# leducthanhig/image-restoration-models

Hardware: AMD Instinct MI355X
Metric: images/sec + PSNR, Restormer motion-deblur 1280x720 (higher is better)
Workload: dtype f32 (1x1 convs: fp32 emulated by 3 fp16 MFMAs on hi/lo operand splits with fp32 accumulation, error vs float64 at the level of an fp32 chain; everything else exact f32; value_exact_f32: f32 MFMA everywhere); 1 GPU; Restormer motion-deblur (WithBias LN, 26.13M params, synthetic weights seed 42) on 1280x720x3 uint8 GoPro-shaped synthetic frames; 6 tiles 512x512 (overlap 96) per frame; a step = 4 frame(s) per GPU, their 24 tiles in one batched forward; global_batch=4, tile=512, overlap=96, parallelism=per-image shard x1, no data-path collective

## Files before the change

### image-restoration-models_amd/csrc/fused_tail.hip

```cpp
#include "irm_common.h"

struct TailArgs {
    const float* Hh; long h_bs;
    float* X; long x_bs;
    const float* rec;
    const float* w2;
    const float* bias2;
    int C, H, W, S, HP, CB;
    float inv_s2;
    int tiles_x, tiles, items, gpx;
};

template <int CT>
__global__ __launch_bounds__(512, 2) void gdfn_tail_kernel(TailArgs a) {
    constexpr int RECF = 512;
    constexpr int W2F = CT * 512, W2P = CT * 2;
    constexpr int SLOT_B = RECF * 4, W2_OFF = 2 * SLOT_B, PL_OFF = W2_OFF + W2F * 4, PL_B = IRM_PLF * 4;
    constexpr int PARK_OFF = PL_OFF + 2 * PL_B;
    constexpr int NK = (IRM_NP * 8 + 511) / 512;
    static_assert(PARK_OFF + 8192 <= 160 * 1024, "LDS");
    extern __shared__ __attribute__((aligned(16))) float smem[];
    irm_lc* lds = (irm_lc*)smem;
    float* slots = smem;
    float* w2a = smem + W2_OFF / 4;

    const int wave = __builtin_amdgcn_readfirstlane((int)threadIdx.x >> 6);
    const long plane = (long)a.H * a.W;
    const int S = a.S;
    const int per = (a.items + 7) >> 3;
    const int xcd = blockIdx.x & 7, pos = blockIdx.x >> 3;
    auto item_of = [&](int round) { const int i = round * a.gpx + pos; return i < per ? xcd * per + i : a.items; };

    int round = 0;
    int item = item_of(0);
    if (item >= a.items) return;

    for (;;) {
        int tid = threadIdx.x;
        asm volatile("" : "+v"(tid));
        const int lane = tid & 63, g = lane >> 4, r = lane & 15;
        const int b = item / a.tiles, tile = item - b * a.tiles;
        const int ty0 = (tile / a.tiles_x) * IRM_TH, tx0 = (tile % a.tiles_x) * IRM_TW;
        const float* Hh = a.Hh + (long)b * a.h_bs;
        const unsigned vw = irm_opaque((unsigned)(lane * 16));
        const unsigned vc = irm_opaque((unsigned)(16 * g));
        const int sp0 = (2 * (wave >> 1)) * IRM_HC + 16 * (wave & 1) + r;
        const unsigned vp0 = irm_opaque((unsigned)(PL_OFF + (sp0 * IRM_PS + 4 * g) * 4));
        const unsigned vp1 = irm_opaque(vp0 + PL_B);

        int goff[NK];
        unsigned loff[NK];
#pragma unroll
        for (int k = 0; k < NK; ++k) {
            const int idx = k * 512 + tid, px = idx >> 3, pc = idx & 7;
            const int hr = px / IRM_HC, hc = px - hr * IRM_HC;
            const int gy = ty0 - 1 + hr, gx = tx0 - 1 + hc;
            const bool valid = px < IRM_NP, inside = valid && gy >= 0 && gy < a.H && gx >= 0 && gx < a.W;
            goff[k] = inside ? ((gy >> 3) * a.tiles_x + (gx >> 5)) * 256 * a.CB + ((gy & 7) * IRM_TW + (gx & 31)) * 64 + (pc & 3) * 4 +
                               (pc >> 2) * (a.HP / 64) * (256 * 64)
                             : -1;
            loff[k] = (unsigned)(PL_OFF + ((valid ? px : IRM_NP + (tid & 15)) * IRM_PS) * 4 + (pc & 3) * 16 + (pc >> 2) * 64);
        }
        f32x4 hreg[NK];
        const float* const zero_page = irm_zero_page;
        auto load_h = [&](int s) {
#pragma unroll
            for (int k = 0; k < NK; ++k) {
                const float* src = goff[k] >= 0 ? Hh + goff[k] + (s >> 2) * (256 * 64) + (s & 3) * 16 : zero_page;
                hreg[k] = *reinterpret_cast<const f32x4*>(src);
            }
        };
        auto park_h = [&](int img) {
#pragma unroll
            for (int k = 0; k < NK; ++k) irm_st<f32x4>(lds, loff[k], img * PL_B, hreg[k]);
        };

        const int nitem = item_of(round + 1);

        irm_dma<2>(a.rec, slots, wave, lane);
        irm_dma<W2P>(a.w2, w2a, wave, lane);
        load_h(0);
        f32x4 acc2[2][CT];
        const unsigned vpark = irm_opaque((unsigned)(PARK_OFF + threadIdx.x * 16));
#pragma unroll
        for (int c = 0; c < CT; ++c) { acc2[0][c] = (f32x4){0.f, 0.f, 0.f, 0.f}; acc2[1][c] = (f32x4){0.f, 0.f, 0.f, 0.f}; }
        irm_st<f32x4>(lds, vpark, 0, acc2[1][CT - 1]);
        park_h(0);
        asm volatile("s_waitcnt vmcnt(0) lgkmcnt(0)" ::: "memory");
        __builtin_amdgcn_s_barrier();

        float o[2][2][4];
        f32x4 kprev[3];

        irm_u4 Gh[2], Gl[2];
#pragma unroll
        for (int q = 0; q < 2; ++q) { Gh[q] = (irm_u4){0u, 0u, 0u, 0u}; Gl[q] = (irm_u4){0u, 0u, 0u, 0u}; }

        auto iter = [&](auto PAR, auto MORE, int it) {
            constexpr int par = decltype(PAR)::value;
            constexpr bool more = decltype(MORE)::value;
            if constexpr (more) {
                load_h(it + 1);
                irm_dma<2>(a.rec + (long)(it + 1) * RECF, slots + (par ^ 1) * RECF, wave, lane);
            }
            if (par == 0 && it > 0) irm_dma<W2P>(a.w2 + (long)(it >> 1) * W2F, w2a, wave, lane);
            {
                const unsigned vp = par ? vp1 : vp0;
                f32x4 P[2][3], K[2][3], KB[1];
                auto loads = [&](auto IC, auto NC) {
                    constexpr int I = decltype(IC)::value, n = decltype(NC)::value;
                    constexpr int hf = I >> 2, dy = I & 3;
                    constexpr int cf = par * SLOT_B + hf * 64;
                    if constexpr (dy == 0) irm_dsr<cf + 9 * 128>(KB[0], vc);
                    if constexpr (dy < 3) {
                        irm_dsr<cf + (dy * 3 + 0) * 128>(K[n][0], vc);
                        irm_dsr<cf + (dy * 3 + 1) * 128>(K[n][1], vc);
                        irm_dsr<cf + (dy * 3 + 2) * 128>(K[n][2], vc);
                    }
                    irm_dsr<(dy * IRM_HC + 0) * (IRM_PS * 4) + hf * 64>(P[n][0], vp);
                    irm_dsr<(dy * IRM_HC + 1) * (IRM_PS * 4) + hf * 64>(P[n][1], vp);
                    irm_dsr<(dy * IRM_HC + 2) * (IRM_PS * 4) + hf * 64>(P[n][2], vp);
                };
                loads(irm_ic<0>{}, irm_ic<0>{});
                irm_for<8>([&](auto IC) {
                    constexpr int I = decltype(IC)::value, c = I & 1, n = c ^ 1;
                    constexpr int hf = I >> 2, dy = I & 3;
                    if constexpr (I + 1 < 8) loads(irm_ic<I + 1>{}, irm_ic<n>{});
                    constexpr int J = I + 1, jdy = J & 3;
                    constexpr int nnext = J < 8 ? 3 + (jdy < 3 ? 3 : 0) + (jdy == 0 ? 1 : 0) : 0;
                    irm_wait_lgkmcnt<nnext>();
                    irm_tie(P[c][0], P[c][1], P[c][2]);
                    if constexpr (dy < 3) irm_tie(K[c][0], K[c][1], K[c][2]);
                    if constexpr (dy == 0) irm_tie(KB[0]);
                    irm_stencil_step(dy, o[hf], kprev, P[c], K[c], KB[0]);
                    __builtin_amdgcn_sched_barrier(0);
                });
            }
#pragma unroll
            for (int q = 0; q < 2; ++q)
#pragma unroll
                for (int e = 0; e < 4; e += 2) {
                    unsigned hh, ll;
                    irm_gate_split2(o[0][q][e], o[0][q][e + 1], o[1][q][e], o[1][q][e + 1], hh, ll);
                    Gh[q][2 * par + e / 2] = hh;
                    Gl[q][2 * par + e / 2] = ll;
                }
#pragma unroll
            for (int q = 0; q < 2; ++q) asm volatile("" : "+v"(Gh[q]), "+v"(Gl[q]));
            if (par == 1 || !more) {
                if constexpr (par == 0) {
                    asm volatile("s_waitcnt vmcnt(0)" ::: "memory");
                    __builtin_amdgcn_s_barrier();
                }
                f32x4 accp = irm_ld<f32x4>(lds, vpark, 0);
#pragma unroll
                for (int c = 0; c < CT; ++c) {
                    const irm_h8 bh = irm_ld<irm_h8>(lds, vw, W2_OFF + (c * 2) * 1024);
                    const irm_h8 bl = irm_ld<irm_h8>(lds, vw, W2_OFF + (c * 2 + 1) * 1024);
#pragma unroll
                    for (int q = 0; q < 2; ++q) {
                        f32x4& t = (q == 1 && c == CT - 1) ? accp : acc2[q][c];
                        t = irm_mfma3_f16(__builtin_bit_cast(irm_h8, Gh[q]), __builtin_bit_cast(irm_h8, Gl[q]), bh, bl, t);
                    }
                }
                irm_st<f32x4>(lds, vpark, 0, accp);
#pragma unroll
                for (int q = 0; q < 2; ++q) { Gh[q] = (irm_u4){0u, 0u, 0u, 0u}; Gl[q] = (irm_u4){0u, 0u, 0u, 0u}; }
            }
            if constexpr (more) park_h(par ^ 1);
            asm volatile("s_waitcnt vmcnt(0) lgkmcnt(0)" ::: "memory");
            __builtin_amdgcn_s_barrier();
        };
        {
            const std::integral_constant<int, 0> P0; const std::integral_constant<int, 1> P1;
            const std::true_type T; const std::false_type F;
            int it = 0;
            for (; it + 2 < S; it += 2) { iter(P0, T, it); iter(P1, T, it + 1); }
            if (it + 2 == S) { iter(P0, T, it); iter(P1, F, it + 1); }
            else iter(P0, F, it);
        }

        {
            int t3 = threadIdx.x;
            asm volatile("" : "+v"(t3));
            const int r3 = t3 & 15, ox = tx0 + 16 * (wave & 1) + 4 * ((t3 & 63) >> 4), oy0 = ty0 + 2 * (wave >> 1);
            float* X = a.X + (long)b * a.x_bs;
            acc2[1][CT - 1] = irm_ld<f32x4>(lds, vpark, 0);
#pragma unroll
            for (int c = 0; c < CT; ++c) {
                const int co = 16 * c + r3;
                if (co >= a.C || ox >= a.W) continue;
                const float bv = a.bias2 ? a.bias2[co] : 0.0f;
#pragma unroll
                for (int q = 0; q < 2; ++q) {
                    if (oy0 + q >= a.H) continue;
                    float4* px = reinterpret_cast<float4*>(X + (long)co * plane + (long)(oy0 + q) * a.W + ox);
                    const float4 xv = *px;
                    *px = make_float4(fmaf(acc2[q][c][0], a.inv_s2, xv.x + bv), fmaf(acc2[q][c][1], a.inv_s2, xv.y + bv),
                                      fmaf(acc2[q][c][2], a.inv_s2, xv.z + bv), fmaf(acc2[q][c][3], a.inv_s2, xv.w + bv));
                }
            }
        }
        if (nitem >= a.items) break;
        item = nitem;
        ++round;
    }
}

extern "C" int irm_gdfn_tail_f16x3_f32(const float* h_cl, long h_bs, const float* rec, const float* w2, const float* bias2,
                                       float* x, long x_bs, float inv_s2, int B, int C, int hid, int hid_pad, int H, int W,
                                       hipStream_t stream) {
    if (!h_cl || !rec || !w2 || !x || B <= 0 || C <= 0 || hid <= 0 || H <= 0 || W <= 0) return IRM_EINVAL;
    if (C != 192 || (H & 7) || (W & 31) || hid_pad < hid || (hid_pad & 63)) return IRM_EINVAL;
    if ((h_bs & 3) || (x_bs & 3) || !irm_aligned16(h_cl) || !irm_aligned16(x) || !irm_aligned16(rec) || !irm_aligned16(w2)) return IRM_EINVAL;
    if ((long)(H / 8) * (W / 32) * 256 * 2 * hid_pad >= (1L << 31)) return IRM_EINVAL;
    TailArgs a;
    a.Hh = h_cl; a.h_bs = h_bs; a.X = x; a.x_bs = x_bs; a.rec = rec; a.w2 = w2; a.bias2 = bias2;
    a.C = C; a.H = H; a.W = W; a.S = (hid + 15) / 16; a.HP = hid_pad; a.CB = 2 * hid_pad; a.inv_s2 = inv_s2;
    a.tiles_x = W / IRM_TW; a.tiles = a.tiles_x * (H / IRM_TH); a.items = B * a.tiles;
    constexpr int CT = 12;
    const size_t lds = (size_t)(2 * 512 + CT * 512 + 2 * IRM_PLF + 2048) * sizeof(float);
    IRM_ALLOW_BIG_LDS((&gdfn_tail_kernel<CT>));
    int dev = 0, n = 0;
    if (hipGetDevice(&dev) != hipSuccess ||
        hipDeviceGetAttribute(&n, hipDeviceAttributeMultiprocessorCount, dev) != hipSuccess || n <= 0) return IRM_ELAUNCH;
    const int per = (a.items + 7) >> 3;
    a.gpx = (n + 7) / 8;
    if (a.gpx > per) a.gpx = per;
    hipLaunchKernelGGL((gdfn_tail_kernel<CT>), dim3(a.gpx * 8), dim3(512), lds, stream, a);
    return irm_launch_status();
}
```

Before: 21.64 images/s.

## Stream GDFN tail halo tiles via direct global-to-LDS loads with triple buffering

Replaces the register-staged load-then-park of the halo hidden tile with global_load_lds DMA into a three-slot LDS ring, issued piecewise between stencil steps and gate math so loads overlap compute across sub-steps and across tile items. Precomputes tile-relative offsets and a boundary class mask once per block instead of per item, and adds an XOR swizzle to the LDS image layout. It also drops the LDS-parked accumulator, keeping all of acc2 in registers, and batches the epilogue's residual loads before the stores. This costs more LDS for the third buffer and more register pressure, and it depends on vmcnt accounting being correct.

```diff
diff --git a/image-restoration-models_amd/csrc/fused_tail.hip b/image-restoration-models_amd/csrc/fused_tail.hip
--- a/image-restoration-models_amd/csrc/fused_tail.hip
+++ b/image-restoration-models_amd/csrc/fused_tail.hip
@@ -11,14 +11,23 @@
     int tiles_x, tiles, items, gpx;
 };
 
+constexpr int TAIL_TAP_B = 512 * 4;
+constexpr int TAIL_HALF_B = IRM_NP * 64, TAIL_IMG_B = 2 * TAIL_HALF_B;
+template <int CT> constexpr int tail_img_off() { return 2 * TAIL_TAP_B + CT * 512 * 4; }
+template <int CT> constexpr int tail_lds_bytes() { return tail_img_off<CT>() + 3 * TAIL_IMG_B; }
+
 template <int CT>
 __global__ __launch_bounds__(512, 2) void gdfn_tail_kernel(TailArgs a) {
     constexpr int RECF = 512;
     constexpr int W2F = CT * 512, W2P = CT * 2;
-    constexpr int SLOT_B = RECF * 4, W2_OFF = 2 * SLOT_B, PL_OFF = W2_OFF + W2F * 4, PL_B = IRM_PLF * 4;
-    constexpr int PARK_OFF = PL_OFF + 2 * PL_B;
-    constexpr int NK = (IRM_NP * 8 + 511) / 512;
-    static_assert(PARK_OFF + 8192 <= 160 * 1024, "LDS");
+    constexpr int SLOT_B = TAIL_TAP_B, W2_OFF = 2 * SLOT_B, PL_OFF = tail_img_off<CT>(), HALF_B = TAIL_HALF_B, PL_B = TAIL_IMG_B;
+    constexpr int NPC = IRM_NP * 8;
+    constexpr int NK = (NPC + 511) / 512;
+    constexpr int PW = (NPC - (NK - 1) * 512) / 8;
+    static_assert(PW * 8 + (NK - 1) * 512 == NPC && PW <= 64, "pieces per wave");
+    static_assert(tail_lds_bytes<CT>() <= 160 * 1024, "LDS");
+    static_assert(NK >= 4 && NK <= 8, "the main loop places four pieces in the stencil and the rest in the gate");
+    static_assert(3 * IRM_HC * 64 + HALF_B < 65536, "stencil read immediates");
     extern __shared__ __attribute__((aligned(16))) float smem[];
     irm_lc* lds = (irm_lc*)smem;
     float* slots = smem;
@@ -35,59 +44,84 @@
     int item = item_of(0);
     if (item >= a.items) return;
 
+    int tid = threadIdx.x;
+    asm volatile("" : "+v"(tid));
+    const int lane = tid & 63, g = lane >> 4, r = lane & 15;
+    const unsigned vw = irm_opaque((unsigned)(lane * 16));
+    const unsigned vc = irm_opaque((unsigned)(16 * g));
+    unsigned vpx[3];
+#pragma unroll
+    for (int dx = 0; dx < 3; ++dx) {
+        const int hc = 16 * (wave & 1) + r + dx;
+        vpx[dx] = irm_opaque((unsigned)(PL_OFF + ((2 * (wave >> 1)) * IRM_HC + hc) * 64 + ((g ^ ((hc >> 1) & 2)) * 16)));
+    }
+
+    unsigned rel[NK], cls = 0;
+#pragma unroll
+    for (int k = 0; k < NK; ++k) {
+        const int idx = k < NK - 1 ? k * 512 + tid : (NK - 1) * 512 + wave * PW + lane;
+        const int hf = idx >= IRM_NP * 4 ? 1 : 0, rem = idx - hf * (IRM_NP * 4), px = rem >> 2;
+        const int hr = px / IRM_HC, hc = px - hr * IRM_HC, q = (rem & 3) ^ ((hc >> 1) & 2);
+        const int ty = hr == 0 ? 0 : hr > IRM_TH ? 2 : 1, py = hr == 0 ? IRM_TH - 1 : hr > IRM_TH ? 0 : hr - 1;
+        const int tx = hc == 0 ? 0 : hc > IRM_TW ? 2 : 1, pxc = hc == 0 ? IRM_TW - 1 : hc > IRM_TW ? 0 : hc - 1;
+        rel[k] = irm_opaque((unsigned)((ty * a.tiles_x + tx) * 256 * a.CB + (py * IRM_TW + pxc) * 64 + q * 4 + hf * (a.HP / 64) * (256 * 64)));
+        cls |= (unsigned)((hr == 0 ? 1 : 0) | (hr > IRM_TH ? 2 : 0) | (hc == 0 ? 4 : 0) | (hc > IRM_TW ? 8 : 0) | 16) << (5 * k);
+    }
+    cls = irm_opaque(cls);
+
+    int rround = 0, rs = 0, rph = 0;
+    const float* rH = a.Hh;
+    unsigned off = 0;
+    auto aim = [&](int it_) {
+        const bool live = it_ < a.items;
+        const int b = live ? it_ / a.tiles : 0, tile = live ? it_ - b * a.tiles : 0;
+        const int ty0 = (tile / a.tiles_x) * IRM_TH, tx0 = (tile % a.tiles_x) * IRM_TW;
+        rH = a.Hh + (long)b * a.h_bs + (long)(tile - a.tiles_x - 1) * (256 * a.CB);
+        const unsigned lacks = (ty0 == 0 ? 1u : 0u) | (ty0 + IRM_TH >= a.H ? 2u : 0u) | (tx0 == 0 ? 4u : 0u) | (tx0 + IRM_TW >= a.W ? 8u : 0u) |
+                               (live ? 0u : 16u);
+        off = cls & (lacks * 0x02108421u);
+    };
+    const float* const zero_page = irm_zero_page;
+    const float* rsrc = rH;
+    irm_lc* rdst = lds;
+    auto req_begin = [&]() {
+        rsrc = rH + (rs >> 2) * (256 * 64) + (rs & 3) * 16;
+        rdst = lds + PL_OFF + rph * PL_B;
+    };
+    auto req_piece = [&](auto KC) {
+        constexpr int k = decltype(KC)::value;
+        const float* src = (off & (31u << (5 * k))) == 0 ? rsrc + rel[k] : zero_page;
+        if constexpr (k < NK - 1)
+            __builtin_amdgcn_global_load_lds((const __attribute__((address_space(1))) void*)src,
+                                             (__attribute__((address_space(3))) void*)(rdst + (k * 512 + wave * 64) * 16), 16, 0, 0);
+        else if (lane < PW)
+            __builtin_amdgcn_global_load_lds((const __attribute__((address_space(1))) void*)src,
+                                             (__attribute__((address_space(3))) void*)(rdst + (k * 512 + wave * PW) * 16), 16, 0, 0);
+    };
+    auto req_end = [&]() {
+        rph = rph == 2 ? 0 : rph + 1;
+        if (++rs == S) { rs = 0; ++rround; aim(item_of(rround)); }
+    };
+    auto request = [&]() { req_begin(); irm_for<NK>(req_piece); req_end(); };
+    auto wait_older = [&]() { asm volatile("s_waitcnt vmcnt(%0) lgkmcnt(0)" ::"n"(NK) : "memory"); };
+
+    int ph = 0;
+    int ts = 0;
+    aim(item);
+    irm_dma<2>(a.rec, slots, wave, lane);
+    request();
+    request();
+    wait_older();
+    __builtin_amdgcn_s_barrier();
+
     for (;;) {
-        int tid = threadIdx.x;
-        asm volatile("" : "+v"(tid));
-        const int lane = tid & 63, g = lane >> 4, r = lane & 15;
         const int b = item / a.tiles, tile = item - b * a.tiles;
         const int ty0 = (tile / a.tiles_x) * IRM_TH, tx0 = (tile % a.tiles_x) * IRM_TW;
-        const float* Hh = a.Hh + (long)b * a.h_bs;
-        const unsigned vw = irm_opaque((unsigned)(lane * 16));
-        const unsigned vc = irm_opaque((unsigned)(16 * g));
-        const int sp0 = (2 * (wave >> 1)) * IRM_HC + 16 * (wave & 1) + r;
-        const unsigned vp0 = irm_opaque((unsigned)(PL_OFF + (sp0 * IRM_PS + 4 * g) * 4));
-        const unsigned vp1 = irm_opaque(vp0 + PL_B);
-
-        int goff[NK];
-        unsigned loff[NK];
-#pragma unroll
-        for (int k = 0; k < NK; ++k) {
-            const int idx = k * 512 + tid, px = idx >> 3, pc = idx & 7;
-            const int hr = px / IRM_HC, hc = px - hr * IRM_HC;
-            const int gy = ty0 - 1 + hr, gx = tx0 - 1 + hc;
-            const bool valid = px < IRM_NP, inside = valid && gy >= 0 && gy < a.H && gx >= 0 && gx < a.W;
-            goff[k] = inside ? ((gy >> 3) * a.tiles_x + (gx >> 5)) * 256 * a.CB + ((gy & 7) * IRM_TW + (gx & 31)) * 64 + (pc & 3) * 4 +
-                               (pc >> 2) * (a.HP / 64) * (256 * 64)
-                             : -1;
-            loff[k] = (unsigned)(PL_OFF + ((valid ? px : IRM_NP + (tid & 15)) * IRM_PS) * 4 + (pc & 3) * 16 + (pc >> 2) * 64);
-        }
-        f32x4 hreg[NK];
-        const float* const zero_page = irm_zero_page;
-        auto load_h = [&](int s) {
-#pragma unroll
-            for (int k = 0; k < NK; ++k) {
-                const float* src = goff[k] >= 0 ? Hh + goff[k] + (s >> 2) * (256 * 64) + (s & 3) * 16 : zero_page;
-                hreg[k] = *reinterpret_cast<const f32x4*>(src);
-            }
-        };
-        auto park_h = [&](int img) {
-#pragma unroll
-            for (int k = 0; k < NK; ++k) irm_st<f32x4>(lds, loff[k], img * PL_B, hreg[k]);
-        };
-
         const int nitem = item_of(round + 1);
 
-        irm_dma<2>(a.rec, slots, wave, lane);
-        irm_dma<W2P>(a.w2, w2a, wave, lane);
-        load_h(0);
         f32x4 acc2[2][CT];
-        const unsigned vpark = irm_opaque((unsigned)(PARK_OFF + threadIdx.x * 16));
 #pragma unroll
         for (int c = 0; c < CT; ++c) { acc2[0][c] = (f32x4){0.f, 0.f, 0.f, 0.f}; acc2[1][c] = (f32x4){0.f, 0.f, 0.f, 0.f}; }
-        irm_st<f32x4>(lds, vpark, 0, acc2[1][CT - 1]);
-        park_h(0);
-        asm volatile("s_waitcnt vmcnt(0) lgkmcnt(0)" ::: "memory");
-        __builtin_amdgcn_s_barrier();
 
         float o[2][2][4];
         f32x4 kprev[3];
@@ -99,27 +133,27 @@
         auto iter = [&](auto PAR, auto MORE, int it) {
             constexpr int par = decltype(PAR)::value;
             constexpr bool more = decltype(MORE)::value;
-            if constexpr (more) {
-                load_h(it + 1);
-                irm_dma<2>(a.rec + (long)(it + 1) * RECF, slots + (par ^ 1) * RECF, wave, lane);
-            }
-            if (par == 0 && it > 0) irm_dma<W2P>(a.w2 + (long)(it >> 1) * W2F, w2a, wave, lane);
+            irm_dma<2>(a.rec + (long)(it + 1 < S ? it + 1 : 0) * RECF, slots + (ts ^ 1) * RECF, wave, lane);
+            if (par == 0) irm_dma<W2P>(a.w2 + (long)(it >> 1) * W2F, w2a, wave, lane);
+            req_begin();
             {
-                const unsigned vp = par ? vp1 : vp0;
+                const unsigned io = (unsigned)(ph * PL_B);
+                const unsigned vq[3] = {irm_opaque(vpx[0] + io), irm_opaque(vpx[1] + io), irm_opaque(vpx[2] + io)};
+                const unsigned vt = irm_opaque(vc + (unsigned)(ts * SLOT_B));
                 f32x4 P[2][3], K[2][3], KB[1];
                 auto loads = [&](auto IC, auto NC) {
                     constexpr int I = decltype(IC)::value, n = decltype(NC)::value;
                     constexpr int hf = I >> 2, dy = I & 3;
-                    constexpr int cf = par * SLOT_B + hf * 64;
-                    if constexpr (dy == 0) irm_dsr<cf + 9 * 128>(KB[0], vc);
+                    constexpr int cf = hf * 64;
+                    if constexpr (dy == 0) irm_dsr<cf + 9 * 128>(KB[0], vt);
                     if constexpr (dy < 3) {
-                        irm_dsr<cf + (dy * 3 + 0) * 128>(K[n][0], vc);
-                        irm_dsr<cf + (dy * 3 + 1) * 128>(K[n][1], vc);
-                        irm_dsr<cf + (dy * 3 + 2) * 128>(K[n][2], vc);
+                        irm_dsr<cf + (dy * 3 + 0) * 128>(K[n][0], vt);
+                        irm_dsr<cf + (dy * 3 + 1) * 128>(K[n][1], vt);
+                        irm_dsr<cf + (dy * 3 + 2) * 128>(K[n][2], vt);
                     }
-                    irm_dsr<(dy * IRM_HC + 0) * (IRM_PS * 4) + hf * 64>(P[n][0], vp);
-                    irm_dsr<(dy * IRM_HC + 1) * (IRM_PS * 4) + hf * 64>(P[n][1], vp);
-                    irm_dsr<(dy * IRM_HC + 2) * (IRM_PS * 4) + hf * 64>(P[n][2], vp);
+                    irm_dsr<dy * IRM_HC * 64 + hf * HALF_B>(P[n][0], vq[0]);
+                    irm_dsr<dy * IRM_HC * 64 + hf * HALF_B>(P[n][1], vq[1]);
+                    irm_dsr<dy * IRM_HC * 64 + hf * HALF_B>(P[n][2], vq[2]);
                 };
                 loads(irm_ic<0>{}, irm_ic<0>{});
                 irm_for<8>([&](auto IC) {
@@ -133,6 +167,7 @@
                     if constexpr (dy < 3) irm_tie(K[c][0], K[c][1], K[c][2]);
                     if constexpr (dy == 0) irm_tie(KB[0]);
                     irm_stencil_step(dy, o[hf], kprev, P[c], K[c], KB[0]);
+                    if constexpr ((I & 1) != 0 && I / 2 < NK) req_piece(irm_ic<I / 2>{});
                     __builtin_amdgcn_sched_barrier(0);
                 });
             }
@@ -144,32 +179,35 @@
                     irm_gate_split2(o[0][q][e], o[0][q][e + 1], o[1][q][e], o[1][q][e + 1], hh, ll);
                     Gh[q][2 * par + e / 2] = hh;
                     Gl[q][2 * par + e / 2] = ll;
+                    if (q == 0 && e == 2) {
+                        __builtin_amdgcn_sched_barrier(0);
+                        irm_for<NK - 4>([&](auto KC) { req_piece(irm_ic<4 + decltype(KC)::value>{}); });
+                        req_end();
+                        __builtin_amdgcn_sched_barrier(0);
+                    }
                 }
 #pragma unroll
             for (int q = 0; q < 2; ++q) asm volatile("" : "+v"(Gh[q]), "+v"(Gl[q]));
             if (par == 1 || !more) {
                 if constexpr (par == 0) {
-                    asm volatile("s_waitcnt vmcnt(0)" ::: "memory");
+                    wait_older();
                     __builtin_amdgcn_s_barrier();
                 }
-                f32x4 accp = irm_ld<f32x4>(lds, vpark, 0);
 #pragma unroll
                 for (int c = 0; c < CT; ++c) {
                     const irm_h8 bh = irm_ld<irm_h8>(lds, vw, W2_OFF + (c * 2) * 1024);
                     const irm_h8 bl = irm_ld<irm_h8>(lds, vw, W2_OFF + (c * 2 + 1) * 1024);
 #pragma unroll
-                    for (int q = 0; q < 2; ++q) {
-                        f32x4& t = (q == 1 && c == CT - 1) ? accp : acc2[q][c];
-                        t = irm_mfma3_f16(__builtin_bit_cast(irm_h8, Gh[q]), __builtin_bit_cast(irm_h8, Gl[q]), bh, bl, t);
-                    }
-                }
-                irm_st<f32x4>(lds, vpark, 0, accp);
+                    for (int q = 0; q < 2; ++q)
+                        acc2[q][c] = irm_mfma3_f16(__builtin_bit_cast(irm_h8, Gh[q]), __builtin_bit_cast(irm_h8, Gl[q]), bh, bl, acc2[q][c]);
+                }
 #pragma unroll
                 for (int q = 0; q < 2; ++q) { Gh[q] = (irm_u4){0u, 0u, 0u, 0u}; Gl[q] = (irm_u4){0u, 0u, 0u, 0u}; }
             }
-            if constexpr (more) park_h(par ^ 1);
-            asm volatile("s_waitcnt vmcnt(0) lgkmcnt(0)" ::: "memory");
+            wait_older();
             __builtin_amdgcn_s_barrier();
+            ph = ph == 2 ? 0 : ph + 1;
+            ts ^= 1;
         };
         {
             const std::integral_constant<int, 0> P0; const std::integral_constant<int, 1> P1;
@@ -184,27 +222,31 @@
             int t3 = threadIdx.x;
             asm volatile("" : "+v"(t3));
             const int r3 = t3 & 15, ox = tx0 + 16 * (wave & 1) + 4 * ((t3 & 63) >> 4), oy0 = ty0 + 2 * (wave >> 1);
-            float* X = a.X + (long)b * a.x_bs;
-            acc2[1][CT - 1] = irm_ld<f32x4>(lds, vpark, 0);
-#pragma unroll
-            for (int c = 0; c < CT; ++c) {
-                const int co = 16 * c + r3;
-                if (co >= a.C || ox >= a.W) continue;
-                const float bv = a.bias2 ? a.bias2[co] : 0.0f;
-#pragma unroll
-                for (int q = 0; q < 2; ++q) {
-                    if (oy0 + q >= a.H) continue;
-                    float4* px = reinterpret_cast<float4*>(X + (long)co * plane + (long)(oy0 + q) * a.W + ox);
-                    const float4 xv = *px;
-                    *px = make_float4(fmaf(acc2[q][c][0], a.inv_s2, xv.x + bv), fmaf(acc2[q][c][1], a.inv_s2, xv.y + bv),
-                                      fmaf(acc2[q][c][2], a.inv_s2, xv.z + bv), fmaf(acc2[q][c][3], a.inv_s2, xv.w + bv));
-                }
+            float* const X = a.X + (long)b * a.x_bs + (long)r3 * plane + (long)oy0 * a.W + ox;
+#pragma unroll
+            for (int c0 = 0; c0 < CT; c0 += CT / 2) {
+                float4 xv[CT / 2][2];
+                float bv[CT / 2];
+#pragma unroll
+                for (int c = 0; c < CT / 2; ++c) {
+                    bv[c] = a.bias2 ? a.bias2[16 * (c0 + c) + r3] : 0.0f;
+#pragma unroll
+                    for (int q = 0; q < 2; ++q) xv[c][q] = *reinterpret_cast<const float4*>(X + (long)(16 * (c0 + c)) * plane + (long)q * a.W);
+                }
+#pragma unroll
+                for (int c = 0; c < CT / 2; ++c)
+#pragma unroll
+                    for (int q = 0; q < 2; ++q)
+                        *reinterpret_cast<float4*>(X + (long)(16 * (c0 + c)) * plane + (long)q * a.W) =
+                            make_float4(fmaf(acc2[q][c0 + c][0], a.inv_s2, xv[c][q].x + bv[c]), fmaf(acc2[q][c0 + c][1], a.inv_s2, xv[c][q].y + bv[c]),
+                                        fmaf(acc2[q][c0 + c][2], a.inv_s2, xv[c][q].z + bv[c]), fmaf(acc2[q][c0 + c][3], a.inv_s2, xv[c][q].w + bv[c]));
             }
         }
         if (nitem >= a.items) break;
         item = nitem;
         ++round;
     }
+    asm volatile("s_waitcnt vmcnt(0)" ::: "memory");
 }
 
 extern "C" int irm_gdfn_tail_f16x3_f32(const float* h_cl, long h_bs, const float* rec, const float* w2, const float* bias2,
@@ -219,7 +261,7 @@
     a.C = C; a.H = H; a.W = W; a.S = (hid + 15) / 16; a.HP = hid_pad; a.CB = 2 * hid_pad; a.inv_s2 = inv_s2;
     a.tiles_x = W / IRM_TW; a.tiles = a.tiles_x * (H / IRM_TH); a.items = B * a.tiles;
     constexpr int CT = 12;
-    const size_t lds = (size_t)(2 * 512 + CT * 512 + 2 * IRM_PLF + 2048) * sizeof(float);
+    const size_t lds = tail_lds_bytes<CT>();
     IRM_ALLOW_BIG_LDS((&gdfn_tail_kernel<CT>));
     int dev = 0, n = 0;
     if (hipGetDevice(&dev) != hipSuccess ||
```

Result: no change. 21.83 images/s (median of 6 runs) (+0.9%).
